# tigert1998/ray-tracing-cuda

Hardware: AMD Instinct MI355X
Metric: Mrays/s (higher is better)
Workload: dtype f32

## Files before the change

ray-tracing-cuda_amd/csrc/closest_hit.h:

```cpp
#pragma once

#ifdef RTMI_CHECK_MARGINS
__device__ inline bool aabb_hit_reference(const BvhNode &nd, V3 o, V3 d, double t_from, double t_to) {
  const float oo[3] = {o.x, o.y, o.z}, dd[3] = {d.x, d.y, d.z};
  for (int i = 0; i < 3; i++) {
    if (dd[i] == 0.f) continue;
    for (int s = 0; s < 2; s++) {
      const float tf = ((s == 0 ? nd.mn[i] : nd.mx[i]) - oo[i]) / dd[i];
      const double t = (double)tf;
      if (t != t || fabs(t) == (double)INFINITY) continue;
      if (!(t_from <= t && t <= t_to)) continue;
      const float pt[3] = {oo[0] + (float)t * dd[0], oo[1] + (float)t * dd[1], oo[2] + (float)t * dd[2]};
      bool inside = true;
      for (int a = 0; a < 3; a++)
        if (a != i && !(nd.mn[a] <= pt[a] && pt[a] <= nd.mx[a])) inside = false;
      if (inside) return true;
    }
  }
  return false;
}
template <typename T>
__device__ inline bool bvh_reference_walk(const SceneDev &sc, const BvhRec &br, V3 o, V3 d, T &t_to, int &face, float &fu,
                                          float &fv) {
  int stk_node[kRefDepthMax + 2], stk_first[kRefDepthMax + 2], stk_n[kRefDepthMax + 2];
// ... 13 lines not shown
        if (tri_test<T>(mk(f.p0[0], f.p0[1], f.p0[2]), mk(f.e1[0], f.e1[1], f.e1[2]), mk(f.e2[0], f.e2[1], f.e2[2]), o, d,
                        t_to, t, u, v))
          t_to = (T)t, face = fi, fu = u, fv = v, hit = true;
      }
    } else if (sp + 2 <= kRefDepthMax + 2) {
      const int mid = (n - 1) / 2;
      stk_node[sp] = nd.right, stk_first[sp] = first + mid + 1, stk_n[sp] = n - mid - 1;
      stk_node[sp + 1] = nd.left, stk_first[sp + 1] = first, stk_n[sp + 1] = mid + 1;
      sp += 2;
    }
  }
  return hit;
}
#endif

template <uint32_t M>
__device__ __forceinline__ bool load_tri_pts(const SceneDev &sc, const float4 *s_tris, int rec, int which, V3 &p0, V3 &e1, V3 &e2) {
  float4 qa, qb, qc;
  bool present;
  if ((M & PIN_LDS_TABLES) || s_tris != nullptr) {
    const float4 *pp = s_tris + (size_t)rec * 3;
    qa = load_lds<float4>(pp), qb = load_lds<float4>(pp + 1), qc = load_lds<float4>(pp + 2);
    present = !(__float_as_int(qc.y) & TRIPTS_ABSENT);
  } else {
    const float4 *pp = reinterpret_cast<const float4 *>(sc.tris + rec);
    qa = load_global<float4>(pp), qb = load_global<float4>(pp + 1), qc = load_global<float4>(pp + 2);
    const float4 qd = load_global<float4>(pp + 3);
    present = which == 0 || (__float_as_int(qd.y) & TRI_SECOND);
  }
  p0 = mk(qa.x, qa.y, qa.z), e1 = mk(qa.w, qb.x, qb.y), e2 = mk(qb.z, qb.w, qc.x);
  return present;
}

template <uint32_t F, bool OCC = false, uint32_t M = 0>
__device__ __forceinline__ Hit closest_hit(const SceneDev &sc, const BvhNode *s_nodes, int lds_nodes, const int *s_paths,
                                           int lds_paths, const float4 *s_tris, int *ll, uint16_t *cands, int *wl,
// ... 14 lines not shown
  float bu = 0.f, bv = 0.f;

  double sa = 0.0, sa2 = 0.0;
  float saf = 0.f;
  if (F & F_SPHERE) {
    float la = len3(d);
    saf = la * la;
    sa = (double)saf;
    sa2 = 2 * sa;
  }

  const int lane = (int)(threadIdx.x & 63u);
  const bool det_safe = (M & PIN_DET_SAFE) || sc.det_safe != 0;
  constexpr bool SLAB = culls_by_slab(M);
  constexpr bool MINF = folds_by_min(M);
  static_assert(!MINF || (!OCC && !DT && !(F & F_TEX)), "a key holds a binary32 t and the triangle's place, nothing else");
  const bool cull_list = (F & F_TRIS) && ((M & PIN_LDS_TABLES) || (ll != nullptr && sc.n_pairs >= kCullMinPairs));
  V3 cull_inv = splat(0.f), cull_klo = splat(0.f), cull_khi = splat(0.f);
  if ((F & F_TRIS) && cull_list) {
    const float ix = __builtin_amdgcn_rcpf(d.x), iy = __builtin_amdgcn_rcpf(d.y), iz = __builtin_amdgcn_rcpf(d.z);
    cull_inv = mk(fabsf(d.x) < 1e-30f ? copysignf(1e30f, d.x) : ix, fabsf(d.y) < 1e-30f ? copysignf(1e30f, d.y) : iy,
                  fabsf(d.z) < 1e-30f ? copysignf(1e30f, d.z) : iz);
    if (SLAB) {
      cull_klo = mk(-o.x * cull_inv.x, -o.y * cull_inv.y, -o.z * cull_inv.z);
    } else {
      const float delta = MESH_DIST_SLACK * (fmaxf(fmaxf(fabsf(o.x), fabsf(o.y)), fabsf(o.z)) + sc.list_mag);
      cull_klo = mk(-(o.x + delta) * cull_inv.x, -(o.y + delta) * cull_inv.y, -(o.z + delta) * cull_inv.z);
      cull_khi = mk(-(o.x - delta) * cull_inv.x, -(o.y - delta) * cull_inv.y, -(o.z - delta) * cull_inv.z);
    }
  }
// ... 64 lines not shown
          __builtin_amdgcn_sched_barrier(0);
          RTMI_CULL_ONE(A)
        }
#undef RTMI_CULL_ONE
#undef RTMI_CULL_SLAB
#undef RTMI_CULL_PAIR
        mask = __brev(mask) >> (32 - nc);
        if (!live) mask = 0u;
        if (OCC && RTMI_DECIDED) mask = 0u;
        RTMI_STAT2(const unsigned long long tc1 = stat_now(); st.cyc[5] += tc1 - tc0;)
        RTMI_STAT(st.cull_bits += (unsigned)__popcll(__builtin_amdgcn_ballot_w64(true)) * 0u; { unsigned pc = __builtin_popcount(mask); for (int off = 32; off > 0; off >>= 1) pc += __shfl_down(pc, off); st.cull_bits += __builtin_amdgcn_readfirstlane(pc); } st.cull_rays += (unsigned)__popcll(__builtin_amdgcn_ballot_w64(true));)
#ifndef RTMI_OWN_FIRST
#define RTMI_OWN_FIRST 1
#endif
#if RTMI_OWN_FIRST
        if (__builtin_amdgcn_ballot_w64(mask != 0u) != 0ull) {
          if (mask != 0u) {
            const int bit = __builtin_ctz(mask);
            mask &= mask - 1u;
            const int rec = 2 * (pair0 + c0 + bit);
            V3 p0, e1, e2, p1, e1b, e2b;
            (void)load_tri_pts<M>(sc, s_tris, rec, 0, p0, e1, e2);
            const bool second = load_tri_pts<M>(sc, s_tris, rec + 1, 1, p1, e1b, e2b);
            float ta = 0.f, ua = 0.f, va = 0.f, tb = 0.f, ub = 0.f, vb = 0.f;
            const bool hit_a = tri_test_flat<T>(p0, e1, e2, cross3(d, e2), o, d, t_to, ta, ua, va, det_safe);
            bool hit_b = false;
            if (second) hit_b = tri_test_flat<T>(p1, e1b, e2b, cross3(d, e2b), o, d, t_to, tb, ub, vb, det_safe) && !hit_a;
            const float t = hit_a ? ta : tb;
            const bool acc = (hit_a || hit_b) && (!ok || (T)t < t_to);
            ok = ok || acc;
            t_to = acc ? (T)t : t_to;
            win = acc ? make_id(RUN_TRIS, run.first + 2 * (c0 + bit) + (hit_a ? 0 : 1)) : win;
            if (F & F_TEX) {
              bu = acc ? (hit_a ? ua : ub) : bu;
              bv = acc ? (hit_a ? va : vb) : bv;
            }
          }
        }
        if (OCC && RTMI_DECIDED) mask = 0u;
#endif
        {
          constexpr int RW = (F & F_TEX) ? 6 : 2;
// ... 1 lines not shown
          const int cnt = __builtin_popcount(mask);
          const int base = wave_prefix_excl(cnt);
          if (cnt != 0) {
            int *rr = ll + lane * 8;
            int w3 = 0, w7 = 0;
            if (DT) {
              const double td = (double)t_to;
              w3 = __double2loint(td), w7 = __double2hiint(td);
            } else {
              w3 = __float_as_int((float)t_to);
            }
            *reinterpret_cast<int4 *>(rr) = make_int4(__float_as_int(o.x), __float_as_int(o.y), __float_as_int(o.z), w3);
            *reinterpret_cast<int4 *>(rr + 4) = make_int4(__float_as_int(d.x), __float_as_int(d.y), __float_as_int(d.z), w7);
          }
          bool todo = cnt != 0;
          while (__builtin_amdgcn_ballot_w64(todo) != 0ull) {
            RTMI_STAT(st.cull_iters++;)
            const int lo_t = __builtin_amdgcn_readlane(base, __builtin_ctzll(__builtin_amdgcn_ballot_w64(todo)));
            const bool now = todo && base + cnt - lo_t <= kListTasks(F);
            const int n_now = __builtin_amdgcn_readlane(base + cnt, 63 - __builtin_clzll(__builtin_amdgcn_ballot_w64(now))) - lo_t;
            RTMI_STAT(st.nnow_hist[(n_now - 1) >> 5 < 5 ? (n_now - 1) >> 5 : 5]++;)
            RTMI_STAT({
              int pc = now ? cnt : 0;
              for (int off = 32; off > 0; off >>= 1) pc = max(pc, __shfl_xor(pc, off));
              st.trip_hist[pc < 8 ? pc - 1 : 7]++;
            })
            int ln = lane;
            if (MINF) asm volatile("" : "+v"(ln));
            if (now) {
              int k = base - lo_t;
              for (uint32_t m = mask; m != 0u; m &= m - 1u) tasks[k++] = (lane << 5) | __builtin_ctz(m);
              if (MINF) results[2 * ln + 1] = -1;
            }
            wave_lds_fence();
            if (MINF) {
              bool flagged = false;
              for (int t0 = 0; t0 < 2 * n_now; t0 += 64) {
                const int ti = t0 + ln;
                if (ti < 2 * n_now) {
                  const int w = tasks[ti >> 1], which = ti & 1;
                  const int *orr = ll + (w >> 5) * 8;
                  const float4 r0 = *reinterpret_cast<const float4 *>(orr), r1 = *reinterpret_cast<const float4 *>(orr + 4);
                  const V3 ro = mk(r0.x, r0.y, r0.z), rd = mk(r1.x, r1.y, r1.z);
                  V3 p0, e1, e2;
                  const bool present = load_tri_pts<M>(sc, s_tris, 2 * (pair0 + c0 + (w & 31)) + which, which, p0, e1, e2);
                  float tt = 0.f, uu, vv;
                  bool hit = false;
                  if (present) hit = tri_test_flat<T>(p0, e1, e2, cross3(rd, e2), ro, rd, (T)r0.w, tt, uu, vv, det_safe);
                  const int mine = hit ? __float_as_int(tt) : -1;
                  const int other = __builtin_amdgcn_update_dpp(mine, mine, 0xb1, 0xf, 0xf, false);
                  const bool yield = other != -1 && (which != 0 || __int_as_float(other) < tt);
                  flagged = flagged || (hit && yield && which == 0);
                  if (hit && !yield) {
                    const unsigned long long key = ((unsigned long long)(uint32_t)mine << 32) | (uint32_t)(2 * (w & 31) + which);
                    (void)__hip_atomic_fetch_min(reinterpret_cast<unsigned long long *>(results + 2 * (w >> 5)), key,
                                                 __ATOMIC_RELAXED, __HIP_MEMORY_SCOPE_WAVEFRONT);
                  }
                }
              }
              wave_lds_fence();
              const unsigned long long fl = __builtin_amdgcn_ballot_w64(flagged);
              if (fl == 0ull) {
                if (now) {
                  const int2 key = *reinterpret_cast<const int2 *>(results + 2 * ln);
                  const float t = __int_as_float(key.y);
                  const bool acc = key.y != -1 && (!ok || (T)t < t_to);
                  ok = ok || acc;
                  t_to = acc ? (T)t : t_to;
                  win = acc ? make_id(RUN_TRIS, run.first + 2 * c0 + key.x) : win;
                  todo = false;
                }
                wave_lds_fence();
                continue;
              }
              if (lane == 0) atomicAdd(overflow + (kOrderedTasksWord - 2), (unsigned long long)__popcll(fl));
            }
            for (int t0 = 0; t0 < 2 * n_now; t0 += 64) {
              const int ti = t0 + lane;
              if (ti < 2 * n_now) {
                const int w = tasks[ti >> 1], which = ti & 1;
                const int *orr = ll + (w >> 5) * 8;
                const float4 r0 = *reinterpret_cast<const float4 *>(orr), r1 = *reinterpret_cast<const float4 *>(orr + 4);
                T t0_to;
                if (DT) {
                  t0_to = (T)__hiloint2double(__float_as_int(r1.w), __float_as_int(r0.w));
                } else {
                  t0_to = (T)r0.w;
                }
                const V3 ro = mk(r0.x, r0.y, r0.z), rd = mk(r1.x, r1.y, r1.z);
                V3 p0, e1, e2;
                const bool present = load_tri_pts<M>(sc, s_tris, 2 * (pair0 + c0 + (w & 31)) + which, which, p0, e1, e2);
                float tt = 0.f, uu = 0.f, vv = 0.f;
                bool hit = false;
                if (present) hit = tri_test_flat<T>(p0, e1, e2, cross3(rd, e2), ro, rd, t0_to, tt, uu, vv, det_safe);
                int *res = results + (ti >> 1) * RW;
                res[which] = hit ? __float_as_int(tt) : (int)0xffffffff;
                if (F & F_TEX) res[2 + 2 * which] = __float_as_int(uu), res[3 + 2 * which] = __float_as_int(vv);
              }
            }
            wave_lds_fence();
            RTMI_STAT2(const unsigned long long tc2 = stat_now();)
            if (now) {
              int k = base - lo_t;
              for (uint32_t m = mask; m != 0u; m &= m - 1u, k++) {
                const int tri = run.first + 2 * (c0 + __builtin_ctz(m));
                const int *res = results + k * RW;
                const int ia = res[0], ib = res[1];
                const float ta = __int_as_float(ia), tb = __int_as_float(ib);
                const bool hit_a = ia != (int)0xffffffff && (T)ta <= t_to;
                const bool hit_b = !hit_a && ib != (int)0xffffffff && (T)tb <= t_to;
                const float t = hit_a ? ta : tb;
                const bool acc = (hit_a || hit_b) && (!ok || (T)t < t_to);
                ok = ok || acc;
                t_to = acc ? (T)t : t_to;
                win = acc ? make_id(RUN_TRIS, tri + (hit_a ? 0 : 1)) : win;
                if (F & F_TEX) {
                  bu = acc ? __int_as_float(hit_a ? res[2] : res[4]) : bu;
                  bv = acc ? __int_as_float(hit_a ? res[3] : res[5]) : bv;
                }
              }
              todo = false;
            }
            wave_lds_fence();
            RTMI_STAT2(st.cyc[7] += stat_now() - tc2;)
          }
        }
        RTMI_STAT2(st.cyc[6] += stat_now() - tc1;)
      }
    } else if ((F & F_TRIS) && live && run.kind == RUN_TRIS) {
      const HotTri *base = sc.tris + run.first;
      f32x16 A = load_hot_tri(base, 0);
      for (int i = 0; i < run.count; i++) {
        if (OCC && __builtin_amdgcn_ballot_w64(!RTMI_DECIDED) == 0ull) break;
        __builtin_amdgcn_s_waitcnt(0xc07f);
        __builtin_amdgcn_sched_barrier(0);
        const f32x16 B = load_hot_tri(base, 2 * i + 1);
        __builtin_amdgcn_sched_barrier(0);
        float t = 0.f, u = 0.f, v = 0.f;
        const V3 pv_a = cross3(d, mk(A[6], A[7], A[8]));
        const bool hit_a = tri_test_flat<T>(mk(A[0], A[1], A[2]), mk(A[3], A[4], A[5]), mk(A[6], A[7], A[8]), pv_a, o, d,
// ... 475 lines not shown
```

ray-tracing-cuda_amd/csrc/kernels.h:

```cpp
#pragma once
#include <hip/hip_runtime.h>
#include <stdint.h>

#include <vector>

#include "../../include/rtmi.h"
#include "scene_dev.h"

#define RTMI_KERNEL_MAX_DEPTH 64

namespace rtmi {

int64_t frame_pixel_of(const FrameDev &fr, int rank, int64_t q);

hipError_t launch_rng_init(uint64_t seed, const FrameDev &fr, const uint32_t *d_jump, uint32_t *d_states,
                           hipStream_t stream, int64_t first = -1);

uint32_t pick_variant(uint32_t features);
int render_occupancy(uint32_t variant, const SceneDev &sc, const FrameDev &fr, int threads, bool fast_path = false);
struct RenderTuning {
  int schedule;
  int blocks_per_cu;
  int threads;
  int sparse_stride;
// ... 19 lines not shown
  PIN_UNSIGNED = 1u << 2,
  PIN_DET_SAFE = 1u << 3,
  PIN_POW2_FRAME = 1u << 4,
  PIN_EVERY_LANE = 1u << 5,
  PIN_PRIORITIES = 1u << 6,
  PIN_CHAINS = 1u << 7,
  PIN_QUEUE = 1u << 8,
};
constexpr uint32_t kFastCommon = PIN_NIBBLE_IDS | PIN_LDS_TABLES | PIN_UNSIGNED | PIN_DET_SAFE | PIN_POW2_FRAME |
                                 PIN_EVERY_LANE | PIN_PRIORITIES;
constexpr uint32_t kFastChains = kFastCommon | PIN_CHAINS;
constexpr uint32_t kFastQueue = kFastCommon | PIN_QUEUE;
constexpr bool defers_unit(uint32_t m) { return (m & kFastCommon) == kFastCommon; }
constexpr bool culls_by_slab(uint32_t m) { return (m & kFastCommon) == kFastCommon; }
constexpr bool folds_by_min(uint32_t m) { return (m & kFastCommon) == kFastCommon; }
constexpr int kOrderedTasksWord = 16;
struct FastPathFacts {
  int enabled;
  uint32_t variant;
  int n_mats;
  int mats_in_lds;
  int pairs_in_lds;
  int unsigned_colours;
  int det_safe;
  int width, height;
  int lane_stride;
  int priorities;
  int chains;
  int resumed;
  int tile_cost;
// ... 126 lines not shown
```

ray-tracing-cuda_amd/csrc/kernels.hip:

```cpp
#include <hip/hip_runtime.h>
#include <stdint.h>

#include "kernels.h"

#include <cfloat>
#include <cmath>
#include <cstdlib>
#include <iterator>
#include <type_traits>
#include "scene_dev.h"
#include "vec.h"
#include "xorwow.h"

namespace rtmi {

__host__ __device__ __forceinline__ int64_t frame_pixel_of_rank(const FrameDev &fr, int rank, int64_t q) {
  int64_t lt = q >> 6;
  int w = (int)(q & 63);
  int64_t gt = lt * fr.world + rank;
  if (gt >= fr.n_tiles) return -1;
  int ty = (int)(gt / fr.tiles_x), tx = (int)(gt % fr.tiles_x);
  int i = ty * 8 + (w >> 3), j = tx * 8 + (w & 7);
  if (i >= fr.height || j >= fr.width) return -1;
  return (int64_t)i * fr.width + j;
// ... 456 lines not shown
  static const bool v = [] {
    const char *e = getenv("RTMI_PLAIN_LIST");
    return e && atoi(e) != 0;
  }();
  return v;
}

static LaunchCfg make_cfg(uint32_t variant, const SceneDev &sc, const FrameDev &fr, int threads, size_t *lds_bytes,
                          bool mats_in_lds = true, bool id_stack = true, bool tex_layers = true) {
  LaunchCfg lc{};
  lc.threads = threads;
  lc.tile_order = nullptr;
  lc.lds_mats = mats_in_lds && sc.n_mats <= kLdsMats ? sc.n_mats : 0;
  lc.wide_ids = sc.n_mats > 256 ? 1 : sc.n_mats <= 16 ? 2 : 0;
  size_t off = ((size_t)lc.lds_mats * sizeof(MatRec) + 15) & ~(size_t)15;
  lc.stack_off = (int32_t)off;
  const size_t levels = (size_t)(fr.max_depth > 0 ? fr.max_depth : 1);
  size_t stack = (variant & F_TEX) && tex_layers ? levels * threads * 4 : (lc.wide_ids == 2 ? (levels + 1) / 2 : levels) * threads * (lc.wide_ids == 1 ? 2 : 1);
  if (!id_stack) stack = 0;
  size_t noff = (off + stack + 15) & ~(size_t)15;
  lc.nodes_off = (int32_t)noff;
  lc.lds_nodes = (variant & F_BVH) ? (sc.n_nodes < kLdsNodes ? sc.n_nodes : kLdsNodes) : 0;
  size_t paoff = (noff + (size_t)lc.lds_nodes * sizeof(BvhNode) + 15) & ~(size_t)15;
  lc.paths_off = (int32_t)paoff;
  lc.lds_paths = (variant & F_BVH) ? (sc.n_leaf_paths < kLdsPaths ? sc.n_leaf_paths : kLdsPaths) : 0;
  size_t soff = (paoff + (size_t)lc.lds_paths * sizeof(int32_t) + 15) & ~(size_t)15;
  lc.mesh_off = (int32_t)soff;
  size_t poff = soff + ((variant & F_BVH) ? (size_t)(threads / 64) * kMeshWaveWords * sizeof(int) : 0);
  const bool cull = (variant & F_TRIS) && sc.n_pairs >= kCullMinPairs && !plain_list_scan();
  const bool staged = cull && sc.n_pairs <= kLdsPairs;
// ... 159 lines not shown
    lc.prio_every = tune.prio_every > 0 ? tune.prio_every : 16;
    {
      const int samples = fr.k_end - fr.k_begin > 0 ? fr.k_end - fr.k_begin : 1;
      const int by_length = 4096 / samples < 1 ? 1 : 4096 / samples;
      lc.fetch_batch = probe && samples <= 4 ? tune.fetch_batch_first : plan.tile_order != nullptr ? std::min(by_length, tune.fetch_batch) : image_order_batch(samples, 16);
    }
    RenderParams rp;
    rp.sc = sc, rp.fr = fr, rp.lc = lc;
    rp.states = d_states, rp.out = d_out, rp.ray_counts = d_ray_counts, rp.counters = d_counters;
    RenderParams *dp = reinterpret_cast<RenderParams *>(d_params);
    const LaunchAt at{blocks, threads, lds, stream};
    if constexpr (F == (uint32_t)F_TRIS) {
      const bool chains = fast == kFastChains && !probe && lc.chain_next && lc.tile_cost && fr.k_begin > 0 && d_ray_counts;
      const bool queue = fast == kFastQueue && !lc.chain_next;
      if (fast != 0u && (!lc.prio_tab || lc.lane_stride != 1 || !(chains || queue))) return hipErrorInvalidValue;
      static_assert(culls_by_slab(kFastChains) && culls_by_slab(kFastQueue) && !culls_by_slab(0u), "which kernels read the slab table");
      if (chains || queue) rp.sc.pair_boxes = pair_slabs_of(sc.pair_boxes, sc.n_pairs);
      if (chains) return launch_block<render_kernel<F, kFastChains>>(at, rp, dp);
      if (queue && !probe) return launch_block<render_kernel<F, kFastQueue>>(at, rp, dp);
      if (queue) return launch_block<probe_kernel<F, kFastQueue>>(at, rp, dp);
    }
    if (fast != 0u) return hipErrorInvalidValue;
    if (probe) return launch_block<probe_kernel<F>>(at, rp, dp);
    return launch_block<render_kernel<F>>(at, rp, dp);
  });
}

hipError_t launch_untile(const FrameDev &fr, const float *d_tiles, float *d_image, hipStream_t stream) {
  int64_t total = fr.items * fr.world;
  if (total == 0) return hipSuccess;
// ... 496 lines not shown
```

ray-tracing-cuda_amd/csrc/render_body.h:

```cpp
#pragma once

struct QueryHit;
template <uint32_t F>
__device__ __forceinline__ QueryHit resolve_hit(const SceneDev &sc, const QueryDev &qd, const Hit &h, V3 o, V3 d);

struct LaunchCfg {
  int32_t lds_mats;
  int32_t wide_ids;
  int32_t stack_off;
  int32_t nodes_off;
  int32_t lds_nodes;
  int32_t mesh_off;
  int32_t exclusive;
  int32_t pairs_off;
  int32_t list_off;
  int32_t paths_off;
  int32_t lds_paths;
  int32_t threads;
  int32_t nrm_off;
  int32_t probe_spp;
  int32_t promote;
  int32_t cand_off;
  const uint32_t *tile_order;
  uint32_t *visit_counts;
// ... 129 lines not shown
                                            const FeatureBufs *feat = nullptr, const StepBufs *step = nullptr,
                                            const ListBufs *list = nullptr) {
  static_assert(!(RAYS && BUDGET), "one work-item source at a time");
  static_assert(!STEP || (RAYS && M == 0), "the step is a mode of the caller's rays");
  static_assert(!LIST || STEP, "the list is where a step's items come from");
  static_assert(!FEATURES || BUDGET, "the feature buffers belong to the budget mode");
  static_assert(M == 0 || (F == F_TRIS && !RAYS && !BUDGET), "the pins are the list-triangle render's");
  static_assert(!((M & PIN_CHAINS) && (M & PIN_QUEUE)), "a wave gets its work one way");
  constexpr bool FOLD4 = (M & (PIN_NIBBLE_IDS | PIN_LDS_TABLES | PIN_UNSIGNED)) == (PIN_NIBBLE_IDS | PIN_LDS_TABLES | PIN_UNSIGNED);
  constexpr bool QUEUE = RAYS || BUDGET;
  extern __shared__ __attribute__((aligned(16))) unsigned char smem[];
  MatRec *s_mats = reinterpret_cast<MatRec *>(smem);
  const uint32_t n_threads = (uint32_t)lc.threads;
  const uint32_t ids_shift = !(M & PIN_NIBBLE_IDS) && lc.wide_ids == 1 ? 1u : 0u;
  const bool nibble_ids = (M & PIN_NIBBLE_IDS) || lc.wide_ids == 2;
  auto ids_offset = [&](int level) -> uint32_t {
    return (uint32_t)lc.stack_off + (((uint32_t)level * n_threads + threadIdx.x) << ids_shift);
  };
  const BvhNode *s_nodes = reinterpret_cast<const BvhNode *>(smem + lc.nodes_off);
  int *wl = nullptr;
  if (F & F_BVH)
    wl = reinterpret_cast<int *>(smem + lc.mesh_off) +
         __builtin_amdgcn_readfirstlane((int)(threadIdx.x >> 6)) * kMeshWaveWords;
  const float4 *s_tris = nullptr;
  if ((F & F_TRIS) && ((M & PIN_LDS_TABLES) || lc.pairs_off >= 0)) {
    s_tris = reinterpret_cast<const float4 *>(smem + lc.pairs_off);
    const uint32_t *src = reinterpret_cast<const uint32_t *>(sc.tri_pts);
    uint32_t *dst = reinterpret_cast<uint32_t *>(smem + lc.pairs_off);
    for (int w = threadIdx.x; w < sc.n_pairs * 24; w += blockDim.x) dst[w] = src[w];
    const uint32_t *nsrc = reinterpret_cast<const uint32_t *>(sc.tri_nrm);
// ... 10 lines not shown
    cands = reinterpret_cast<uint16_t *>(smem + lc.cand_off) +
            __builtin_amdgcn_readfirstlane((int)(threadIdx.x >> 6)) * (64 * kSphCand + 128);
  const bool mats_in_lds = (M & PIN_LDS_TABLES) || lc.lds_mats > 0;
  auto lds_rgb = [&](int m) -> V3 {
    const float4 c = load_lds<float4>(s_mats + m);
    return mk(c.x, c.y, c.z);
  };
  auto lds_byte = [&](uint32_t byte_offset) -> uint32_t {
    return *(const RT_LDS uint8_t *)(uintptr_t)byte_offset;
  };
  const bool fast_fold = FOLD4 || (mats_in_lds && lc.wide_ids != 1 && sc.unsigned_colours);
  if (mats_in_lds) {
    const uint32_t *src = reinterpret_cast<const uint32_t *>(sc.mats);
    uint32_t *dst = reinterpret_cast<uint32_t *>(s_mats);
    for (int w = threadIdx.x; w < lc.lds_mats * 8; w += blockDim.x) dst[w] = src[w];
  }
  if ((F & F_BVH) && lc.lds_nodes > 0) {
    const uint32_t *src = reinterpret_cast<const uint32_t *>(sc.nodes);
    uint32_t *dst = reinterpret_cast<uint32_t *>(smem + lc.nodes_off);
    for (int w = threadIdx.x; w < lc.lds_nodes * 8; w += blockDim.x) dst[w] = src[w];
  }
  const int *s_paths = reinterpret_cast<const int *>(smem + lc.paths_off);
  if ((F & F_BVH) && lc.lds_paths > 0) {
    int *dst = reinterpret_cast<int *>(smem + lc.paths_off);
    for (int w = threadIdx.x; w < lc.lds_paths; w += blockDim.x) dst[w] = sc.leaf_paths[w];
  }
  __syncthreads();

  const int64_t n_items = fr.items;
  const bool w_pow2 = (fr.width & (fr.width - 1)) == 0, h_pow2 = (fr.height & (fr.height - 1)) == 0;
  const double inv_w = 1.0 / (double)fr.width, inv_h = 1.0 / (double)fr.height;
// ... 57 lines not shown
        if constexpr (!STEP) {
          out[q * 3 + 0] = 0.f, out[q * 3 + 1] = 0.f, out[q * 3 + 2] = 0.f;
          if (ray_counts) ray_counts[q] = 0;
        }
        return false;
      }
      o = ro, d = nd;
    }
    int64_t idx = RAYS ? 0 : frame_pixel_of_rank(fr, fr.rank, q);
    if constexpr (BUDGET) {
      if (idx < 0) return false;
      const uint32_t b = budget[q];
      k_end_px = (int)(b < (uint32_t)fr.spp ? b : (uint32_t)fr.spp);
      if (k_end_px <= 0) return false;
    } else if (idx < 0 || fr.spp <= 0) {
      out[q * 3 + 0] = 0.f, out[q * 3 + 1] = 0.f, out[q * 3 + 2] = 0.f;
      if ((M & PIN_CHAINS) || ray_counts) ray_counts[q] = 0;
      return false;
    }
    if (!RAYS) pij = ((uint32_t)(idx / fr.width) << 16) | (uint32_t)(idx % fr.width);
    rng.d = states[0 * n_items + q];
    rng.v0 = states[1 * n_items + q];
    rng.v1 = states[2 * n_items + q];
    rng.v2 = states[3 * n_items + q];
    rng.v3 = states[4 * n_items + q];
    rng.v4 = states[5 * n_items + q];
    k = fr.k_begin;
    rays = 0;
    work_px = 0;
    color = splat(0.f);
    if ((M & PIN_CHAINS) || fr.k_begin > 0) {
// ... 264 lines not shown
          }
        }
        o = origin;
        d = DEFER ? target - origin : unit3_rn_twice(target - origin);
        k++;
        if ((F & F_BVH) && promote && cls == 1 && k >= lc.promote) {
          const unsigned long long have = (unsigned long long)rays * (unsigned)lc.probe_spp, per = (unsigned long long)k;
          if (have >= thr16 * per) cls = have >= thr64 * per ? 64 : have >= thr32 * per ? 32 : 16;
        }
        depth = DEFER ? kOwesBit : 0;
        active = true;
      }
    }
    if constexpr (DEFER) {
      if (depth < 0) {
        d = unit3_rn_twice(d);
        depth &= ~kOwesBit;
      }
    }
    if (!__any(active)) {
      if (!(F & F_BVH) || __all(done)) break;
      continue;
    }

#if defined(RTMI_STATS) && RTMI_STATS == 9
    if ((wave_queries + 1u) % 600u == 0u && (wave_queries + 1u) / 600u <= 9u && (threadIdx.x & 63u) == 0u)
      g_wave_stats[((blockIdx.x * blockDim.x + threadIdx.x) >> 6) & 16383u][(wave_queries + 1u) / 600u] =
          ((stat_real() - t_begin) & 0xffffffffffull) | ((unsigned long long)(st.node_steps + st.face_steps) << 40);
#endif
    RTMI_STAT(wave_queries++; const unsigned long long tq1 = stat_now(); st.cyc[0] += tq1 - tq0;
              const unsigned long long in0 = st.cyc[2] + st.cyc[3];)
// ... 30 lines not shown
#ifdef RTMI_STATS
                           , st
#endif
        );
      rays++;
      if ((F & F_BVH) && lc.visit_counts != nullptr) work_px += (uint32_t)h.work;

      V3 result = splat(0.f);
      bool ended = true;
      V3 step_att = splat(0.f), step_o = o, step_d = splat(0.f);
      if (h.ok && depth < fr.max_depth) {
        const uint32_t kind = h.win >> 29;
        const uint32_t index = h.win & ID_INDEX_MASK;
        V3 p = o + h.t * d;
        if (kind == RUN_SKY) {
          V3 dir = unit3_rn(p);
          float tg = (float)(0.5 * ((double)dir.y + 1.0));
          float w0 = 1.0f - tg;
          result = mk(w0 * 1.0f + tg * 0.5f, w0 * 1.0f + tg * 0.7f, w0 * 1.0f + tg * 1.0f);
          if constexpr (FEATURES) {
            if (depth == 0 && feat->albedo) feature_add3(feat->albedo, result);
          }
        } else {
          V3 nrm = splat(0.f);
          int mat = 0;
          float tu = 0.f, tv = 0.f;
          if ((F & F_TRIS) && kind == RUN_TRIS) {
            V3 n;
            int flags;
            if ((M & PIN_LDS_TABLES) || s_tris != nullptr) {
              const float4 tn = s_nrm[index];
// ... 73 lines not shown
              if (feat->normal) feature_add3(feat->normal, nrm);
              if (feat->depth) feat->depth[q32] = __fadd_rn(feat->depth[q32], h.t);
              if (feat->coverage) feat->coverage[q32] += 1u;
            }
          }
          if (m.kind == MAT_LIGHT) {
            result = rgb;
          } else {
            const float dn = dot3(d, nrm);
            V3 nd = splat(0.f);
            bool scattered = false;
            if (m.kind == MAT_LAMBERTIAN) {
              if (!(dn >= 0.f)) {
                float sum;
                V3 s = ball_sample(rng, sum);
                s = sampler_on_sphere(s, sum);
                nd = STEP ? unit3_rn(s + nrm) : DEFER ? s + nrm : unit3_rn_twice(s + nrm);
                scattered = true;
              }
            } else if (m.kind == MAT_METAL) {
              if (!(dn >= 0.f)) {
                V3 refl = reflect3(d, nrm);
                if (m.param > 0.f) {
                  float sum;
                  V3 s = ball_sample(rng, sum);
                  nd = refl + m.param * s;
                } else {
                  nd = refl;
                }
                if (!STEP) nd = unit3_rn(nd);
                scattered = true;
              }
            } else {
              if (dn >= 0.f)
                nd = refract3(d, -nrm, m.param / 1.0f);
              else
                nd = refract3(d, nrm, 1.0f / m.param);
              bool zero = (nd.x == 0.f && nd.y == 0.f && nd.z == 0.f);
              bool nan = (nd.x != nd.x) || (nd.y != nd.y) || (nd.z != nd.z);
              scattered = !(zero || nan);
              if (!STEP && scattered) nd = unit3_rn(nd);
            }
            if constexpr (STEP) {
              if (scattered) {
                step_att = ((F & F_TEX) && (layer >> 31)) ? texel_rgb(layer) : rgb;
                step_o = p, step_d = nd;
                ended = false;
              }
            }
            if (!STEP && scattered) {
              if (tex32) {
                *reinterpret_cast<uint32_t *>(smem + tex_layer_offset(depth)) = layer;
              } else if (nibble_ids) {
                const uint32_t at = ids_offset(depth >> 1);
                const uint32_t old = smem[at];
                smem[at] = (uint8_t)((depth & 1) ? ((old & 0x0fu) | ((uint32_t)mat << 4)) : ((old & 0xf0u) | (uint32_t)mat));
// ... 35 lines not shown
          rec[0] = make_int4(__float_as_int(r.t), __float_as_int(r.u), __float_as_int(r.v), __float_as_int(r.n.x));
          rec[1] = make_int4(__float_as_int(r.n.y), __float_as_int(r.n.z), r.mat, r.kind);
          rec[2] = make_int4(r.entry, r.element, 0, 0);
        }
        if (step->steps) step->steps[q] += 1u;
        ray_acc += 1u;
        active = false, has_px = false;
        ended = false;
      }
      if (ended) {
        int i = depth - 1;
        if (!tex32 && fast_fold) {
          const uint32_t step = n_threads;
          if (nibble_ids) {
            uint32_t at = ids_offset(i >= 0 ? i >> 1 : 0);
            if (i >= 0 && !(i & 1)) {
              const int m0 = lds_byte(at) & 15;
              { const V3 a_ = lds_rgb(m0); result = mk(a_.x * result.x, a_.y * result.y, a_.z * result.z); }
              i--, at -= step;
            }
            for (; i >= 3; i -= 4, at -= 2u * step) {
              const uint32_t b0 = lds_byte(at), b1 = lds_byte(at - step);
              const int m0 = b0 >> 4, m1 = b0 & 15, m2 = b1 >> 4, m3 = b1 & 15;
              const V3 a0 = lds_rgb(m0), a1 = lds_rgb(m1);
              const V3 a2 = lds_rgb(m2), a3 = lds_rgb(m3);
              result = mk(a0.x * result.x, a0.y * result.y, a0.z * result.z);
              result = mk(a1.x * result.x, a1.y * result.y, a1.z * result.z);
              result = mk(a2.x * result.x, a2.y * result.y, a2.z * result.z);
              result = mk(a3.x * result.x, a3.y * result.y, a3.z * result.z);
            }
            for (; i >= 1; i -= 2, at -= step) {
              const uint32_t b0 = lds_byte(at);
              const int m0 = b0 >> 4, m1 = b0 & 15;
              { const V3 a_ = lds_rgb(m0); result = mk(a_.x * result.x, a_.y * result.y, a_.z * result.z); }
              { const V3 a_ = lds_rgb(m1); result = mk(a_.x * result.x, a_.y * result.y, a_.z * result.z); }
            }
          } else {
            uint32_t at = ids_offset(i >= 0 ? i : 0);
            for (; i >= 3; i -= 4, at -= 4u * step) {
              const int m0 = lds_byte(at), m1 = lds_byte(at - step), m2 = lds_byte(at - 2u * step), m3 = lds_byte(at - 3u * step);
              const V3 a0 = lds_rgb(m0), a1 = lds_rgb(m1);
              const V3 a2 = lds_rgb(m2), a3 = lds_rgb(m3);
              result = mk(a0.x * result.x, a0.y * result.y, a0.z * result.z);
              result = mk(a1.x * result.x, a1.y * result.y, a1.z * result.z);
              result = mk(a2.x * result.x, a2.y * result.y, a2.z * result.z);
              result = mk(a3.x * result.x, a3.y * result.y, a3.z * result.z);
            }
            for (; i >= 0; i--, at -= step) {
              const int m0 = lds_byte(at);
              { const V3 a_ = lds_rgb(m0); result = mk(a_.x * result.x, a_.y * result.y, a_.z * result.z); }
// ... 88 lines not shown
```

ray-tracing-cuda_amd/csrc/trace_helpers.h:

```cpp
#pragma once

template <bool DT>
struct TSel {
  typedef float type;
};
template <>
struct TSel<true> {
  typedef double type;
};

constexpr uint32_t ID_NONE = 0xffffffffu;
constexpr uint32_t ID_INDEX_MASK = (1u << 28) - 1;
__device__ __forceinline__ uint32_t make_id(int kind, int index) { return ((uint32_t)kind << 29) | (uint32_t)index; }

#define T_FROM_F 0.001f
#define DET_EPS_F 1e-7f

#define RCP_RN_LIMIT 0x1p126f
__device__ __forceinline__ float rcp_rn(float x) {
  const float r = __builtin_amdgcn_rcpf(x);
  const float e = __builtin_fmaf(-x, r, 1.0f);
  return __builtin_fmaf(e, r, r);
}

#define SQRT_RN_LO 0x1p-100f
#define SQRT_RN_HI 0x1p100f
__device__ __forceinline__ float sqrt_rn_core(float x) {
  const float y = __builtin_amdgcn_rsqf(x);
  const float g = x * y, h = 0.5f * y;
  const float d = __builtin_fmaf(-g, g, x);
  return __builtin_fmaf(d, h, g);
}
#ifndef RTMI_OPT_SQRT
#define RTMI_OPT_SQRT 1
#endif
#ifndef RTMI_OPT_DIV3
#define RTMI_OPT_DIV3 1
#endif
__device__ __forceinline__ float sqrt_rn(float x) {
#if RTMI_OPT_SQRT
  if (__all(x >= SQRT_RN_LO && x < SQRT_RN_HI)) return sqrt_rn_core(x);
#endif
  return sqrtf(x);
}

#define DIV3_RN_LO 0x1p-40f
__device__ __forceinline__ float div_rn_core(float a, float b, float y) {
  float q = a * y;
  q = __builtin_fmaf(__builtin_fmaf(-b, q, a), y, q);
  q = __builtin_fmaf(__builtin_fmaf(-b, q, a), y, q);
  return q;
}
__device__ __forceinline__ V3 sampler_on_sphere(V3 a, float sum) {
#if RTMI_OPT_DIV3
  if (__all(sum >= 0x1p-80f)) {
    const float l = sqrt_rn_core(sum);
    const float y = rcp_rn(l);
    return mk(div_rn_core(a.x, l, y), div_rn_core(a.y, l, y), div_rn_core(a.z, l, y));
  }
  const float l = sqrtf(sum);
#else
  const float l = sqrt_rn(sum);
#endif
  return mk(a.x / l, a.y / l, a.z / l);
}

__device__ __forceinline__ V3 unit3_rn(V3 v) {
  const float dd = dot3(v, v);
  float inv;
#if RTMI_OPT_SQRT
  if (__all(dd >= SQRT_RN_LO && dd < SQRT_RN_HI)) {
    inv = rcp_rn(sqrt_rn_core(dd));
  } else {
    inv = 1.0f / sqrtf(dd);
  }
#else
  const float s = sqrtf(dd);
  if (__all(__builtin_amdgcn_class(s, 0x100))) {
    inv = rcp_rn(s);
  } else {
    inv = 1.0f / s;
  }
#endif
  return v * inv;
}

__device__ __forceinline__ V3 unit3_rn_twice(V3 v) {
#if RTMI_OPT_SQRT
  const float dd = dot3(v, v);
  if (__all(dd >= SQRT_RN_LO && dd < SQRT_RN_HI)) {
    const V3 u = v * rcp_rn(sqrt_rn_core(dd));
    return u * rcp_rn(sqrt_rn_core(dot3(u, u)));
  }
  const V3 u = v * (1.0f / sqrtf(dd));
  return u * (1.0f / sqrtf(dot3(u, u)));
#else
  return unit3_rn(unit3_rn(v));
#endif
}

template <typename T>
__device__ __forceinline__ bool tri_test(V3 p0, V3 e1, V3 e2, V3 o, V3 d, T t_to, float &t, float &u, float &v) {
  V3 pvec = cross3(d, e2);
  float det = dot3(e1, pvec);
  if (fabsf(det) < DET_EPS_F) return false;
  float inv;
  if (fabsf(det) < RCP_RN_LIMIT) {
    inv = rcp_rn(det);
  } else {
    inv = 1.0f / det;
  }
  V3 tvec = o - p0;
  u = dot3(tvec, pvec) * inv;
  if (u < 0.0f || u > 1.0f) return false;
  V3 qvec = cross3(tvec, e1);
  v = dot3(d, qvec) * inv;
  if (v < 0.0f || u + v > 1.0f) return false;
  t = dot3(e2, qvec) * inv;
  if (!(T_FROM_F <= t && (T)t <= t_to)) return false;
  return true;
}
template <typename T>
__device__ __forceinline__ bool tri_test_flat(V3 p0, V3 e1, V3 e2, V3 pvec, V3 o, V3 d, T t_to, float &t, float &u,
                                              float &v, bool det_safe = false) {
  float det = dot3(e1, pvec);
  bool ok = !(fabsf(det) < DET_EPS_F);
  float inv;
  if (det_safe || __all(fabsf(det) < RCP_RN_LIMIT)) {
    inv = rcp_rn(det);
  } else {
    inv = 1.0f / det;
  }
  V3 tvec = o - p0;
  u = dot3(tvec, pvec) * inv;
  ok = ok & !((u < 0.0f) | (u > 1.0f));
  V3 qvec = cross3(tvec, e1);
  v = dot3(d, qvec) * inv;
  ok = ok & !((v < 0.0f) | (u + v > 1.0f));
  t = dot3(e2, qvec) * inv;
  ok = ok & ((T_FROM_F <= t) & ((T)t <= t_to));
  return ok;
}

// ... 154 lines not shown
```

Baseline: 36980.

## Trim wave votes, use 24-bit LDS addressing, and fold material RGB table

Replaces ballot/all-based wave votes with single compare intrinsics (icmp/fcmp returning a lane mask), computes staged triangle LDS addresses with a 24-bit multiply, and stages a compact 16-byte-per-row RGB table in LDS so nibble material ids index colour directly in the throughput fold. The aim is to trim scalar/vector instructions in hot loops of the fast-path kernels. It adds a fixed LDS layout requirement for the fast path (launch rejects other stack offsets), which may fail configurations that were valid before.

```diff
diff --git a/ray-tracing-cuda_amd/csrc/closest_hit.h b/ray-tracing-cuda_amd/csrc/closest_hit.h
--- a/ray-tracing-cuda_amd/csrc/closest_hit.h
+++ b/ray-tracing-cuda_amd/csrc/closest_hit.h
@@ -51,12 +51,17 @@
 }
 #endif
 
-template <uint32_t M>
+template <uint32_t M, bool PAIR = false>
 __device__ __forceinline__ bool load_tri_pts(const SceneDev &sc, const float4 *s_tris, int rec, int which, V3 &p0, V3 &e1, V3 &e2) {
   float4 qa, qb, qc;
   bool present;
   if ((M & PIN_LDS_TABLES) || s_tris != nullptr) {
     const float4 *pp = s_tris + (size_t)rec * 3;
+    if (trims_mul24(M)) {
+      uint32_t at = (uint32_t)(uintptr_t)s_tris + __umul24((uint32_t)(PAIR ? rec - which : rec), 48u);
+      asm volatile("" : "+v"(at));
+      pp = (const float4 *)(const RT_LDS float4 *)(uintptr_t)at + (PAIR ? 3 * which : 0);
+    }
     qa = load_lds<float4>(pp), qb = load_lds<float4>(pp + 1), qc = load_lds<float4>(pp + 2);
     present = !(__float_as_int(qc.y) & TRIPTS_ABSENT);
   } else {
@@ -101,6 +106,7 @@
   const bool det_safe = (M & PIN_DET_SAFE) || sc.det_safe != 0;
   constexpr bool SLAB = culls_by_slab(M);
   constexpr bool MINF = folds_by_min(M);
+  constexpr bool VOTE = trims_votes(M);
   static_assert(!MINF || (!OCC && !DT && !(F & F_TEX)), "a key holds a binary32 t and the triangle's place, nothing else");
   const bool cull_list = (F & F_TRIS) && ((M & PIN_LDS_TABLES) || (ll != nullptr && sc.n_pairs >= kCullMinPairs));
   V3 cull_inv = splat(0.f), cull_klo = splat(0.f), cull_khi = splat(0.f);
@@ -195,18 +201,18 @@
 #define RTMI_OWN_FIRST 1
 #endif
 #if RTMI_OWN_FIRST
-        if (__builtin_amdgcn_ballot_w64(mask != 0u) != 0ull) {
+        if (wave_ballot_nz<VOTE>(mask) != 0ull) {
           if (mask != 0u) {
             const int bit = __builtin_ctz(mask);
             mask &= mask - 1u;
             const int rec = 2 * (pair0 + c0 + bit);
             V3 p0, e1, e2, p1, e1b, e2b;
-            (void)load_tri_pts<M>(sc, s_tris, rec, 0, p0, e1, e2);
-            const bool second = load_tri_pts<M>(sc, s_tris, rec + 1, 1, p1, e1b, e2b);
+            (void)load_tri_pts<M, true>(sc, s_tris, rec, 0, p0, e1, e2);
+            const bool second = load_tri_pts<M, true>(sc, s_tris, rec + 1, 1, p1, e1b, e2b);
             float ta = 0.f, ua = 0.f, va = 0.f, tb = 0.f, ub = 0.f, vb = 0.f;
-            const bool hit_a = tri_test_flat<T>(p0, e1, e2, cross3(d, e2), o, d, t_to, ta, ua, va, det_safe);
+            const bool hit_a = tri_test_flat<T, VOTE>(p0, e1, e2, cross3(d, e2), o, d, t_to, ta, ua, va, det_safe);
             bool hit_b = false;
-            if (second) hit_b = tri_test_flat<T>(p1, e1b, e2b, cross3(d, e2b), o, d, t_to, tb, ub, vb, det_safe) && !hit_a;
+            if (second) hit_b = tri_test_flat<T, VOTE>(p1, e1b, e2b, cross3(d, e2b), o, d, t_to, tb, ub, vb, det_safe) && !hit_a;
             const float t = hit_a ? ta : tb;
             const bool acc = (hit_a || hit_b) && (!ok || (T)t < t_to);
             ok = ok || acc;
@@ -238,11 +244,15 @@
             *reinterpret_cast<int4 *>(rr + 4) = make_int4(__float_as_int(d.x), __float_as_int(d.y), __float_as_int(d.z), w7);
           }
           bool todo = cnt != 0;
-          while (__builtin_amdgcn_ballot_w64(todo) != 0ull) {
+          uint32_t left = (uint32_t)cnt;
+#define RTMI_TODO_LANES (VOTE ? wave_ballot_nz<true>(left) : __builtin_amdgcn_ballot_w64(todo))
+          while (RTMI_TODO_LANES != 0ull) {
             RTMI_STAT(st.cull_iters++;)
-            const int lo_t = __builtin_amdgcn_readlane(base, __builtin_ctzll(__builtin_amdgcn_ballot_w64(todo)));
-            const bool now = todo && base + cnt - lo_t <= kListTasks(F);
-            const int n_now = __builtin_amdgcn_readlane(base + cnt, 63 - __builtin_clzll(__builtin_amdgcn_ballot_w64(now))) - lo_t;
+            const int lo_t = __builtin_amdgcn_readlane(base, __builtin_ctzll(RTMI_TODO_LANES));
+            const bool now = (VOTE ? left != 0u : todo) && base + cnt - lo_t <= kListTasks(F);
+            const unsigned long long now_lanes = VOTE ? RTMI_TODO_LANES & __builtin_amdgcn_sicmp(base + cnt - lo_t, kListTasks(F), 41)
+                                                      : __builtin_amdgcn_ballot_w64(now);
+            const int n_now = __builtin_amdgcn_readlane(base + cnt, 63 - __builtin_clzll(now_lanes)) - lo_t;
             RTMI_STAT(st.nnow_hist[(n_now - 1) >> 5 < 5 ? (n_now - 1) >> 5 : 5]++;)
             RTMI_STAT({
               int pc = now ? cnt : 0;
@@ -270,7 +280,7 @@
                   const bool present = load_tri_pts<M>(sc, s_tris, 2 * (pair0 + c0 + (w & 31)) + which, which, p0, e1, e2);
                   float tt = 0.f, uu, vv;
                   bool hit = false;
-                  if (present) hit = tri_test_flat<T>(p0, e1, e2, cross3(rd, e2), ro, rd, (T)r0.w, tt, uu, vv, det_safe);
+                  if (present) hit = tri_test_flat<T, VOTE>(p0, e1, e2, cross3(rd, e2), ro, rd, (T)r0.w, tt, uu, vv, det_safe);
                   const int mine = hit ? __float_as_int(tt) : -1;
                   const int other = __builtin_amdgcn_update_dpp(mine, mine, 0xb1, 0xf, 0xf, false);
                   const bool yield = other != -1 && (which != 0 || __int_as_float(other) < tt);
@@ -292,7 +302,7 @@
                   ok = ok || acc;
                   t_to = acc ? (T)t : t_to;
                   win = acc ? make_id(RUN_TRIS, run.first + 2 * c0 + key.x) : win;
-                  todo = false;
+                  todo = false, left = 0u;
                 }
                 wave_lds_fence();
                 continue;
@@ -316,7 +326,7 @@
                 const bool present = load_tri_pts<M>(sc, s_tris, 2 * (pair0 + c0 + (w & 31)) + which, which, p0, e1, e2);
                 float tt = 0.f, uu = 0.f, vv = 0.f;
                 bool hit = false;
-                if (present) hit = tri_test_flat<T>(p0, e1, e2, cross3(rd, e2), ro, rd, t0_to, tt, uu, vv, det_safe);
+                if (present) hit = tri_test_flat<T, VOTE>(p0, e1, e2, cross3(rd, e2), ro, rd, t0_to, tt, uu, vv, det_safe);
                 int *res = results + (ti >> 1) * RW;
                 res[which] = hit ? __float_as_int(tt) : (int)0xffffffff;
                 if (F & F_TEX) res[2 + 2 * which] = __float_as_int(uu), res[3 + 2 * which] = __float_as_int(vv);
@@ -343,11 +353,12 @@
                   bv = acc ? __int_as_float(hit_a ? res[3] : res[5]) : bv;
                 }
               }
-              todo = false;
+              todo = false, left = 0u;
             }
             wave_lds_fence();
             RTMI_STAT2(st.cyc[7] += stat_now() - tc2;)
           }
+#undef RTMI_TODO_LANES
         }
         RTMI_STAT2(st.cyc[6] += stat_now() - tc1;)
       }
diff --git a/ray-tracing-cuda_amd/csrc/kernels.h b/ray-tracing-cuda_amd/csrc/kernels.h
--- a/ray-tracing-cuda_amd/csrc/kernels.h
+++ b/ray-tracing-cuda_amd/csrc/kernels.h
@@ -57,6 +57,14 @@
 constexpr bool defers_unit(uint32_t m) { return (m & kFastCommon) == kFastCommon; }
 constexpr bool culls_by_slab(uint32_t m) { return (m & kFastCommon) == kFastCommon; }
 constexpr bool folds_by_min(uint32_t m) { return (m & kFastCommon) == kFastCommon; }
+#ifndef RTMI_TRIM
+#define RTMI_TRIM 7
+#endif
+constexpr bool trims_votes(uint32_t m) { return (RTMI_TRIM & 1) && (m & kFastCommon) == kFastCommon; }
+constexpr bool trims_mul24(uint32_t m) { return (RTMI_TRIM & 2) && (m & kFastCommon) == kFastCommon; }
+constexpr bool trims_fold_rgb(uint32_t m) { return (RTMI_TRIM & 4) && (m & kFastCommon) == kFastCommon; }
+constexpr int kFoldRgbOff = 512;
+constexpr int kFoldRgbBytes = 256;
 constexpr int kOrderedTasksWord = 16;
 struct FastPathFacts {
   int enabled;
diff --git a/ray-tracing-cuda_amd/csrc/kernels.hip b/ray-tracing-cuda_amd/csrc/kernels.hip
--- a/ray-tracing-cuda_amd/csrc/kernels.hip
+++ b/ray-tracing-cuda_amd/csrc/kernels.hip
@@ -494,6 +494,10 @@
   lc.lds_mats = mats_in_lds && sc.n_mats <= kLdsMats ? sc.n_mats : 0;
   lc.wide_ids = sc.n_mats > 256 ? 1 : sc.n_mats <= 16 ? 2 : 0;
   size_t off = ((size_t)lc.lds_mats * sizeof(MatRec) + 15) & ~(size_t)15;
+  static_assert(kFoldRgbOff == 16 * sizeof(MatRec) && kFoldRgbOff % 16 == 0, "behind the largest table nibble ids can name");
+  if (variant == (uint32_t)F_TRIS && lc.wide_ids == 2 && lc.lds_mats > 0 && id_stack) off = (size_t)kFoldRgbOff + kFoldRgbBytes;
+  static_assert((uint64_t)(2 * kLdsPairs + 2) * sizeof(TriPts) < (1u << 24) && sizeof(TriPts) == 48,
+                "staged TriPts records: index (one pair of padding included) x 48 bytes is a 24-bit product");
   lc.stack_off = (int32_t)off;
   const size_t levels = (size_t)(fr.max_depth > 0 ? fr.max_depth : 1);
   size_t stack = (variant & F_TEX) && tex_layers ? levels * threads * 4 : (lc.wide_ids == 2 ? (levels + 1) / 2 : levels) * threads * (lc.wide_ids == 1 ? 2 : 1);
@@ -683,6 +687,7 @@
       const bool chains = fast == kFastChains && !probe && lc.chain_next && lc.tile_cost && fr.k_begin > 0 && d_ray_counts;
       const bool queue = fast == kFastQueue && !lc.chain_next;
       if (fast != 0u && (!lc.prio_tab || lc.lane_stride != 1 || !(chains || queue))) return hipErrorInvalidValue;
+      if (fast != 0u && lc.stack_off != kFoldRgbOff + kFoldRgbBytes) return hipErrorInvalidValue;
       static_assert(culls_by_slab(kFastChains) && culls_by_slab(kFastQueue) && !culls_by_slab(0u), "which kernels read the slab table");
       if (chains || queue) rp.sc.pair_boxes = pair_slabs_of(sc.pair_boxes, sc.n_pairs);
       if (chains) return launch_block<render_kernel<F, kFastChains>>(at, rp, dp);
diff --git a/ray-tracing-cuda_amd/csrc/render_body.h b/ray-tracing-cuda_amd/csrc/render_body.h
--- a/ray-tracing-cuda_amd/csrc/render_body.h
+++ b/ray-tracing-cuda_amd/csrc/render_body.h
@@ -167,6 +167,8 @@
   const uint32_t n_threads = (uint32_t)lc.threads;
   const uint32_t ids_shift = !(M & PIN_NIBBLE_IDS) && lc.wide_ids == 1 ? 1u : 0u;
   const bool nibble_ids = (M & PIN_NIBBLE_IDS) || lc.wide_ids == 2;
+  constexpr bool VOTE = trims_votes(M), FOLD_RGB = trims_fold_rgb(M);
+  static_assert(!FOLD_RGB || ((M & PIN_NIBBLE_IDS) && (M & PIN_LDS_TABLES)), "the table's rows are named by nibbles and staged with the materials");
   auto ids_offset = [&](int level) -> uint32_t {
     return (uint32_t)lc.stack_off + (((uint32_t)level * n_threads + threadIdx.x) << ids_shift);
   };
@@ -207,7 +209,17 @@
     const uint32_t *src = reinterpret_cast<const uint32_t *>(sc.mats);
     uint32_t *dst = reinterpret_cast<uint32_t *>(s_mats);
     for (int w = threadIdx.x; w < lc.lds_mats * 8; w += blockDim.x) dst[w] = src[w];
+    if constexpr (FOLD_RGB) {
+      uint32_t *rgb = reinterpret_cast<uint32_t *>(smem + kFoldRgbOff);
+      for (int w = threadIdx.x; w < kFoldRgbBytes / 4; w += blockDim.x)
+        rgb[w] = (w & 3) != 3 && (w >> 2) < lc.lds_mats ? src[(w >> 2) * 8 + (w & 3)] : 0u;
+    }
   }
+  auto fold_rgb = [&](uint32_t row16) -> V3 {
+    typedef float f32x3 __attribute__((ext_vector_type(3)));
+    const f32x3 c = *(const RT_LDS f32x3 *)(uintptr_t)((uint32_t)kFoldRgbOff + row16);
+    return mk(c[0], c[1], c[2]);
+  };
   if ((F & F_BVH) && lc.lds_nodes > 0) {
     const uint32_t *src = reinterpret_cast<const uint32_t *>(sc.nodes);
     uint32_t *dst = reinterpret_cast<uint32_t *>(smem + lc.nodes_off);
@@ -295,7 +307,9 @@
       k_end_px = (int)(b < (uint32_t)fr.spp ? b : (uint32_t)fr.spp);
       if (k_end_px <= 0) return false;
     } else if (idx < 0 || fr.spp <= 0) {
-      out[q * 3 + 0] = 0.f, out[q * 3 + 1] = 0.f, out[q * 3 + 2] = 0.f;
+      float zero = 0.f;
+      if constexpr (VOTE || FOLD_RGB) asm volatile("" : "+v"(zero));
+      out[q * 3 + 0] = zero, out[q * 3 + 1] = zero, out[q * 3 + 2] = zero;
       if ((M & PIN_CHAINS) || ray_counts) ray_counts[q] = 0;
       return false;
     }
@@ -590,7 +604,7 @@
     }
     if constexpr (DEFER) {
       if (depth < 0) {
-        d = unit3_rn_twice(d);
+        d = unit3_rn_twice<VOTE>(d);
         depth &= ~kOwesBit;
       }
     }
@@ -651,7 +665,7 @@
         const uint32_t index = h.win & ID_INDEX_MASK;
         V3 p = o + h.t * d;
         if (kind == RUN_SKY) {
-          V3 dir = unit3_rn(p);
+          V3 dir = unit3_rn<VOTE>(p);
           float tg = (float)(0.5 * ((double)dir.y + 1.0));
           float w0 = 1.0f - tg;
           result = mk(w0 * 1.0f + tg * 0.5f, w0 * 1.0f + tg * 0.7f, w0 * 1.0f + tg * 1.0f);
@@ -755,8 +769,8 @@
               if (!(dn >= 0.f)) {
                 float sum;
                 V3 s = ball_sample(rng, sum);
-                s = sampler_on_sphere(s, sum);
-                nd = STEP ? unit3_rn(s + nrm) : DEFER ? s + nrm : unit3_rn_twice(s + nrm);
+                s = sampler_on_sphere<VOTE>(s, sum);
+                nd = STEP ? unit3_rn(s + nrm) : DEFER ? s + nrm : unit3_rn_twice<VOTE>(s + nrm);
                 scattered = true;
               }
             } else if (m.kind == MAT_METAL) {
@@ -769,7 +783,7 @@
                 } else {
                   nd = refl;
                 }
-                if (!STEP) nd = unit3_rn(nd);
+                if (!STEP) nd = unit3_rn<VOTE>(nd);
                 scattered = true;
               }
             } else {
@@ -780,7 +794,7 @@
               bool zero = (nd.x == 0.f && nd.y == 0.f && nd.z == 0.f);
               bool nan = (nd.x != nd.x) || (nd.y != nd.y) || (nd.z != nd.z);
               scattered = !(zero || nan);
-              if (!STEP && scattered) nd = unit3_rn(nd);
+              if (!STEP && scattered) nd = unit3_rn<VOTE>(nd);
             }
             if constexpr (STEP) {
               if (scattered) {
@@ -846,26 +860,47 @@
           const uint32_t step = n_threads;
           if (nibble_ids) {
             uint32_t at = ids_offset(i >= 0 ? i >> 1 : 0);
-            if (i >= 0 && !(i & 1)) {
-              const int m0 = lds_byte(at) & 15;
-              { const V3 a_ = lds_rgb(m0); result = mk(a_.x * result.x, a_.y * result.y, a_.z * result.z); }
-              i--, at -= step;
-            }
-            for (; i >= 3; i -= 4, at -= 2u * step) {
-              const uint32_t b0 = lds_byte(at), b1 = lds_byte(at - step);
-              const int m0 = b0 >> 4, m1 = b0 & 15, m2 = b1 >> 4, m3 = b1 & 15;
-              const V3 a0 = lds_rgb(m0), a1 = lds_rgb(m1);
-              const V3 a2 = lds_rgb(m2), a3 = lds_rgb(m3);
-              result = mk(a0.x * result.x, a0.y * result.y, a0.z * result.z);
-              result = mk(a1.x * result.x, a1.y * result.y, a1.z * result.z);
-              result = mk(a2.x * result.x, a2.y * result.y, a2.z * result.z);
-              result = mk(a3.x * result.x, a3.y * result.y, a3.z * result.z);
-            }
-            for (; i >= 1; i -= 2, at -= step) {
-              const uint32_t b0 = lds_byte(at);
-              const int m0 = b0 >> 4, m1 = b0 & 15;
-              { const V3 a_ = lds_rgb(m0); result = mk(a_.x * result.x, a_.y * result.y, a_.z * result.z); }
-              { const V3 a_ = lds_rgb(m1); result = mk(a_.x * result.x, a_.y * result.y, a_.z * result.z); }
+            if constexpr (FOLD_RGB) {
+              if (i >= 0 && !(i & 1)) {
+                { const V3 a_ = fold_rgb((lds_byte(at) << 4) & 0xf0u); result = mk(a_.x * result.x, a_.y * result.y, a_.z * result.z); }
+                i--, at -= step;
+              }
+              for (; i >= 3; i -= 4, at -= 2u * step) {
+                const uint32_t b0 = lds_byte(at), b1 = lds_byte(at - step);
+                const V3 a0 = fold_rgb(b0 & 0xf0u), a1 = fold_rgb((b0 << 4) & 0xf0u);
+                const V3 a2 = fold_rgb(b1 & 0xf0u), a3 = fold_rgb((b1 << 4) & 0xf0u);
+                result = mk(a0.x * result.x, a0.y * result.y, a0.z * result.z);
+                result = mk(a1.x * result.x, a1.y * result.y, a1.z * result.z);
+                result = mk(a2.x * result.x, a2.y * result.y, a2.z * result.z);
+                result = mk(a3.x * result.x, a3.y * result.y, a3.z * result.z);
+              }
+              for (; i >= 1; i -= 2, at -= step) {
+                const uint32_t b0 = lds_byte(at);
+                { const V3 a_ = fold_rgb(b0 & 0xf0u); result = mk(a_.x * result.x, a_.y * result.y, a_.z * result.z); }
+                { const V3 a_ = fold_rgb((b0 << 4) & 0xf0u); result = mk(a_.x * result.x, a_.y * result.y, a_.z * result.z); }
+              }
+            } else {
+              if (i >= 0 && !(i & 1)) {
+                const int m0 = lds_byte(at) & 15;
+                { const V3 a_ = lds_rgb(m0); result = mk(a_.x * result.x, a_.y * result.y, a_.z * result.z); }
+                i--, at -= step;
+              }
+              for (; i >= 3; i -= 4, at -= 2u * step) {
+                const uint32_t b0 = lds_byte(at), b1 = lds_byte(at - step);
+                const int m0 = b0 >> 4, m1 = b0 & 15, m2 = b1 >> 4, m3 = b1 & 15;
+                const V3 a0 = lds_rgb(m0), a1 = lds_rgb(m1);
+                const V3 a2 = lds_rgb(m2), a3 = lds_rgb(m3);
+                result = mk(a0.x * result.x, a0.y * result.y, a0.z * result.z);
+                result = mk(a1.x * result.x, a1.y * result.y, a1.z * result.z);
+                result = mk(a2.x * result.x, a2.y * result.y, a2.z * result.z);
+                result = mk(a3.x * result.x, a3.y * result.y, a3.z * result.z);
+              }
+              for (; i >= 1; i -= 2, at -= step) {
+                const uint32_t b0 = lds_byte(at);
+                const int m0 = b0 >> 4, m1 = b0 & 15;
+                { const V3 a_ = lds_rgb(m0); result = mk(a_.x * result.x, a_.y * result.y, a_.z * result.z); }
+                { const V3 a_ = lds_rgb(m1); result = mk(a_.x * result.x, a_.y * result.y, a_.z * result.z); }
+              }
             }
           } else {
             uint32_t at = ids_offset(i >= 0 ? i : 0);
diff --git a/ray-tracing-cuda_amd/csrc/trace_helpers.h b/ray-tracing-cuda_amd/csrc/trace_helpers.h
--- a/ray-tracing-cuda_amd/csrc/trace_helpers.h
+++ b/ray-tracing-cuda_amd/csrc/trace_helpers.h
@@ -31,15 +31,37 @@
   const float d = __builtin_fmaf(-g, g, x);
   return __builtin_fmaf(d, h, g);
 }
+template <bool ONE>
+__device__ __forceinline__ unsigned long long wave_ballot_nz(uint32_t v) {
+  if constexpr (ONE) return __builtin_amdgcn_uicmp(v, 0u, 33);
+  else return __builtin_amdgcn_ballot_w64(v != 0u);
+}
+template <bool ONE>
+__device__ __forceinline__ bool wave_all_in(float x, float lo, float hi) {
+  if constexpr (ONE) return (__builtin_amdgcn_fcmpf(x, lo, 12) | __builtin_amdgcn_fcmpf(x, hi, 11)) == 0ull;
+  else return __all(x >= lo && x < hi);
+}
+template <bool ONE>
+__device__ __forceinline__ bool wave_all_ge(float x, float lo) {
+  if constexpr (ONE) return __builtin_amdgcn_fcmpf(x, lo, 12) == 0ull;
+  else return __all(x >= lo);
+}
+template <bool ONE>
+__device__ __forceinline__ bool wave_all_lt(float x, float hi) {
+  if constexpr (ONE) return __builtin_amdgcn_fcmpf(x, hi, 11) == 0ull;
+  else return __all(x < hi);
+}
+
 #ifndef RTMI_OPT_SQRT
 #define RTMI_OPT_SQRT 1
 #endif
 #ifndef RTMI_OPT_DIV3
 #define RTMI_OPT_DIV3 1
 #endif
+template <bool ONE = false>
 __device__ __forceinline__ float sqrt_rn(float x) {
 #if RTMI_OPT_SQRT
-  if (__all(x >= SQRT_RN_LO && x < SQRT_RN_HI)) return sqrt_rn_core(x);
+  if (wave_all_in<ONE>(x, SQRT_RN_LO, SQRT_RN_HI)) return sqrt_rn_core(x);
 #endif
   return sqrtf(x);
 }
@@ -51,25 +73,27 @@
   q = __builtin_fmaf(__builtin_fmaf(-b, q, a), y, q);
   return q;
 }
+template <bool ONE = false>
 __device__ __forceinline__ V3 sampler_on_sphere(V3 a, float sum) {
 #if RTMI_OPT_DIV3
-  if (__all(sum >= 0x1p-80f)) {
+  if (wave_all_ge<ONE>(sum, 0x1p-80f)) {
     const float l = sqrt_rn_core(sum);
     const float y = rcp_rn(l);
     return mk(div_rn_core(a.x, l, y), div_rn_core(a.y, l, y), div_rn_core(a.z, l, y));
   }
   const float l = sqrtf(sum);
 #else
-  const float l = sqrt_rn(sum);
+  const float l = sqrt_rn<ONE>(sum);
 #endif
   return mk(a.x / l, a.y / l, a.z / l);
 }
 
+template <bool ONE = false>
 __device__ __forceinline__ V3 unit3_rn(V3 v) {
   const float dd = dot3(v, v);
   float inv;
 #if RTMI_OPT_SQRT
-  if (__all(dd >= SQRT_RN_LO && dd < SQRT_RN_HI)) {
+  if (wave_all_in<ONE>(dd, SQRT_RN_LO, SQRT_RN_HI)) {
     inv = rcp_rn(sqrt_rn_core(dd));
   } else {
     inv = 1.0f / sqrtf(dd);
@@ -85,17 +109,18 @@
   return v * inv;
 }
 
+template <bool ONE = false>
 __device__ __forceinline__ V3 unit3_rn_twice(V3 v) {
 #if RTMI_OPT_SQRT
   const float dd = dot3(v, v);
-  if (__all(dd >= SQRT_RN_LO && dd < SQRT_RN_HI)) {
+  if (wave_all_in<ONE>(dd, SQRT_RN_LO, SQRT_RN_HI)) {
     const V3 u = v * rcp_rn(sqrt_rn_core(dd));
     return u * rcp_rn(sqrt_rn_core(dot3(u, u)));
   }
   const V3 u = v * (1.0f / sqrtf(dd));
   return u * (1.0f / sqrtf(dot3(u, u)));
 #else
-  return unit3_rn(unit3_rn(v));
+  return unit3_rn<ONE>(unit3_rn<ONE>(v));
 #endif
 }
 
@@ -120,13 +145,13 @@
   if (!(T_FROM_F <= t && (T)t <= t_to)) return false;
   return true;
 }
-template <typename T>
+template <typename T, bool ONE = false>
 __device__ __forceinline__ bool tri_test_flat(V3 p0, V3 e1, V3 e2, V3 pvec, V3 o, V3 d, T t_to, float &t, float &u,
                                               float &v, bool det_safe = false) {
   float det = dot3(e1, pvec);
   bool ok = !(fabsf(det) < DET_EPS_F);
   float inv;
-  if (det_safe || __all(fabsf(det) < RCP_RN_LIMIT)) {
+  if (det_safe || wave_all_lt<ONE>(fabsf(det), RCP_RN_LIMIT)) {
     inv = rcp_rn(det);
   } else {
     inv = 1.0f / det;
```

Result: faster. 38560 (median of 6 runs) (+4.3%).
